# acappemin/Video-to-Audio-and-Piano-RP

Measured on AMD Instinct MI355X. Metric: mel-frames/sec (10s VGGSound shape, 32-step CFM, CFG 2.0), higher is better.
Workload: dtype bf16x3; 1 GPU; BASELINE.json configs[1]: 1 clip(s)/GPU x 750 latent frames x 128 ch, 32-point sway grid = 31 CFG evaluations (62 DiT forwards), T5 context 16 tokens, V2A zero roll; clips_per_gpu=1, global_clips=1, parallelism=clip-sharded x1, 1 all-gather, hipgraph=True, schedule=three streams, side_streams=True, cascade_passes=1

## Files before the change

video-to-audio-and-piano-rp_amd/csrc/gemm_common.h:

```cpp
#pragma once
#include "v2a_common.h"
#include <stdlib.h>
#include <type_traits>

namespace v2a_detail {

struct GemmParams {
  const void* a[3];
  int64_t lda[3];
  int32_t kend[3];
  int32_t nseg;
  const void* w;
  int64_t ldw;
  const float* bias;
  int32_t M, N, K;
  void* out;
  int64_t ldo;
  bf16_t* out2;
  int64_t ldo2;
  const float* resid;
  int64_t ldr;
  const float* gate;
  const int32_t* step;
  int64_t gss, gbs;
  int32_t rpb;
  const float* rope;
  int32_t rope_cols, rope_pos_off;
  int32_t vec_epi;
  int32_t relu;
  const int32_t* a_rowoff;
  const int32_t* a_koff;
  const int32_t* o_rowoff;
  int32_t krot;
  const float* ngam;
  int64_t ngss, ngbs;
  int32_t nsw_row, nsw_off;
  float* ssq;
  int64_t ssq_ld;
  const float* rssq;
  int64_t rssq_ld;
  int32_t rssq_parts;
  float rnorm;
  int32_t xcd_gm, xcd_gn;
  struct Rect { int32_t m_lo, n_lo, cnt, hm; float rcp; } rect[8];
  int32_t nrect, tiles_m, tiles_n;
  int32_t out2_split, out_split;
  int64_t alo[3];
  int64_t out2_lo;
  int32_t s3_kl;
  int32_t dbg;
};

struct GemmTuning {
  int force_tile;
  int krot;
  int use_8phase;
  int min_tiles_8phase;
  int xcd_grid;
  int dbg;
};
extern GemmTuning g_gemm_tuning;
extern int g_attn_one_group_from;
extern int g_dwconv_rows_per_wave;
extern int g_probe_dbg;
extern int g_dwconv_stream;

int launch_gemm_8phase(const GemmParams& p, int epilogue, int out_dtype, hipStream_t stream);

inline void fill_tile_map(GemmParams& p, int BM, int BN) {
  p.tiles_m = (p.M + BM - 1) / BM;
  p.tiles_n = (p.N + BN - 1) / BN;
  const int gm = p.xcd_gm, gn = p.xcd_gn;
  p.nrect = gm * gn;
  for (int r = 0; r < p.nrect; ++r) {
    const int xm = r / gn, xn = r % gn;
    const int m_lo = xm * p.tiles_m / gm, m_hi = (xm + 1) * p.tiles_m / gm;
    const int n_lo = xn * p.tiles_n / gn, n_hi = (xn + 1) * p.tiles_n / gn;
    const int hm = m_hi - m_lo;
    p.rect[r].m_lo = m_lo;
    p.rect[r].n_lo = n_lo;
    p.rect[r].cnt = hm * (n_hi - n_lo);
    p.rect[r].hm = hm > 0 ? hm : 1;
    p.rect[r].rcp = 1.0f / (float)(hm > 0 ? hm : 1);
  }
}

}

namespace {

using v2a_detail::GemmParams;

__device__ __forceinline__ void tile_of_index(const GemmParams& p, int L, int& tm, int& tn) {
  tm = tn = 0;
#pragma unroll
  for (int r = 0; r < 8; ++r) {
    if (r < p.nrect) {
      const int cnt = p.rect[r].cnt;
      if (L >= 0 && L < cnt) {
        const int hm = p.rect[r].hm;
        int q = (int)((float)L * p.rect[r].rcp);
        int rem = L - q * hm;
        if (rem < 0) { --q; rem += hm; }
        else if (rem >= hm) { ++q; rem -= hm; }
        tn = p.rect[r].n_lo + q;
        tm = p.rect[r].m_lo + rem;
      }
      L -= cnt;
    }
  }
}
__device__ __forceinline__ void tile_of_block(const GemmParams& p, int bid, int& tm, int& tn) {
  const int nwg = p.tiles_m * p.tiles_n;
  const int q = nwg >> 3, r = nwg & 7, xcd = bid & 7;
  const int L = (xcd < r ? xcd * (q + 1) : r * (q + 1) + (xcd - r) * q) + (bid >> 3);
  tile_of_index(p, L, tm, tn);
}

__host__ __device__ constexpr bool is_glu(int epi) { return epi == V2A_EPI_GEGLU || epi == V2A_EPI_SWIGLU; }
template <int EPI, bool FAST> __device__ __forceinline__ float glu_act(float g) {
  if constexpr (EPI == V2A_EPI_SWIGLU) return FAST ? silu_f(g) : silu_exact_f(g);
  else return FAST ? gelu_fast_f(g) : gelu_erf_f(g);
}

template <typename T> struct TileCfg;
template <> struct TileCfg<bf16_t> {
  static constexpr int BK = 64;
  static constexpr int LDS_ROW = 64;
};
template <> struct TileCfg<float> {
  static constexpr int BK = 16;
  static constexpr int LDS_ROW = 20;
};

template <int ROWS, bool SRC_F32> struct StageBf16 {
  static constexpr int N = ROWS / 32;
  bf16x8 r[N];
  __device__ __forceinline__ void load(const void* base, int64_t ld, int row0, int rows_total, int k0, int tid) {
    const int chunk = tid & 7;
#pragma unroll
    for (int i = 0; i < N; ++i) {
      int row = row0 + (tid >> 3) + 32 * i;
      row = row < rows_total ? row : rows_total - 1;
      if constexpr (SRC_F32) {
        const float* p = reinterpret_cast<const float*>(base) + (int64_t)row * ld + k0 + chunk * 8;
        f32x4 lo = *reinterpret_cast<const f32x4*>(p);
        f32x4 hi = *reinterpret_cast<const f32x4*>(p + 4);
        bf16x8 v;
#pragma unroll
        for (int j = 0; j < 4; ++j) {
          v[j] = (bf16_t)lo[j];
          v[4 + j] = (bf16_t)hi[j];
        }
        r[i] = v;
      } else {
        const bf16_t* p = reinterpret_cast<const bf16_t*>(base) + (int64_t)row * ld + k0 + chunk * 8;
        r[i] = *reinterpret_cast<const bf16x8*>(p);
      }
    }
  }
  __device__ __forceinline__ void store(bf16_t* lds, int tid) const {
    const int chunk = tid & 7;
#pragma unroll
    for (int i = 0; i < N; ++i) {
      int row = (tid >> 3) + 32 * i;
      *reinterpret_cast<bf16x8*>(lds + row * 64 + ((chunk ^ (row & 7)) << 3)) = r[i];
    }
  }
};

template <int ROWS> struct StageF32 {
  static constexpr int N = ROWS / 64;
  f32x4 r[N];
  __device__ __forceinline__ void load(const void* base, int64_t ld, int row0, int rows_total, int k0, int tid) {
    const int c4 = tid & 3;
#pragma unroll
    for (int i = 0; i < N; ++i) {
      int row = row0 + (tid >> 2) + 64 * i;
      row = row < rows_total ? row : rows_total - 1;
      const float* p = reinterpret_cast<const float*>(base) + (int64_t)row * ld + k0 + c4 * 4;
      r[i] = *reinterpret_cast<const f32x4*>(p);
    }
  }
  __device__ __forceinline__ void store(float* lds, int tid) const {
    const int c4 = tid & 3;
#pragma unroll
    for (int i = 0; i < N; ++i) {
      int row = (tid >> 2) + 64 * i;
      *reinterpret_cast<f32x4*>(lds + row * 20 + c4 * 4) = r[i];
    }
  }
};

template <typename T, bool A_F32, int ROWS> struct StageSel;
template <bool A_F32, int ROWS> struct StageSel<bf16_t, A_F32, ROWS> { using type = StageBf16<ROWS, A_F32>; };
template <bool A_F32, int ROWS> struct StageSel<float, A_F32, ROWS> { using type = StageF32<ROWS>; };

template <int EPI, typename OutT, int TM, int TN, int WM, int WN>
__device__ __forceinline__ void gemm_epilogue(const GemmParams& p, f32x4 (&acc)[TM][TN], int m0, int n0, int wm, int wn,
                                              int lr, int lq) {
  OutT* out = reinterpret_cast<OutT*>(p.out);
#pragma unroll
  for (int i = 0; i < TM; ++i) {
#pragma unroll
    for (int jj = 0; jj < 4; ++jj) {
      const int m = m0 + wm * WM + i * 16 + lq * 4 + jj;
      if (m >= p.M) continue;
      const float* gvec = nullptr;
      if constexpr (EPI == V2A_EPI_GATE_RESID) gvec = step_vec(p.gate, p.step, p.gss, p.gbs, p.gbs ? m / p.rpb : 0);
      if constexpr (is_glu(EPI)) {
#pragma unroll
        for (int j = 0; j < TN; j += 2) {
          const int n = n0 + wn * WN + j * 16 + lr;
          if (n >= p.N) continue;
          float v = acc[i][j][jj], g = acc[i][j + 1][jj];
          if (p.bias) { v += p.bias[n]; g += p.bias[n + 16]; }
          const int oc = ((n0 + wn * WN) >> 1) + (j >> 1) * 16 + lr;
          const float ge = glu_act<EPI, sizeof(OutT) == 2>(g);
          out[(int64_t)m * p.ldo + oc] = from_f32<OutT>(v * ge);
        }
      } else {
#pragma unroll
        for (int j = 0; j < TN; ++j) {
          const int n = n0 + wn * WN + j * 16 + lr;
          if (n >= p.N) continue;
          float v = acc[i][j][jj];
          if (p.bias) v += p.bias[n];
          if constexpr (EPI == V2A_EPI_SIGMOID) v = sigmoid_f(v);
          if constexpr (EPI == V2A_EPI_GELU) v = gelu_erf_f(v);
          if constexpr (EPI == V2A_EPI_RESID) v += p.resid[(int64_t)m * p.ldr + n];
          if constexpr (EPI == V2A_EPI_GATE_RESID) v = p.resid[(int64_t)m * p.ldr + n] + gvec[n] * v;
          if (p.relu) v = fmaxf(v, 0.f);
          out[(int64_t)m * p.ldo + n] = from_f32<OutT>(v);
          if constexpr (sizeof(OutT) == 4) {
            if (p.out2) p.out2[(int64_t)m * p.ldo2 + n] = (bf16_t)v;
          }
        }
      }
    }
  }
}


template <int EPI, int TM, int WN, bool ON> struct EpiPrefetch {
  static constexpr int LPR = WN / 4, RPI = 64 / LPR, RPS = 16 / RPI;
  static constexpr bool RES = ON && (EPI == V2A_EPI_RESID || EPI == V2A_EPI_GATE_RESID);
  static constexpr bool GATE = ON && EPI == V2A_EPI_GATE_RESID;
  f32x4 rs[RES ? TM : 1][RES ? RPS : 1];
  f32x4 gt[GATE ? TM : 1][GATE ? RPS : 1];
  static constexpr bool SCAT = RES && !GATE;
  int32_t ro[SCAT ? TM : 1][SCAT ? RPS : 1];
  static constexpr bool ROPE = ON && EPI == V2A_EPI_STORE;
  f32x4 cs[ROPE ? TM : 1][ROPE ? RPS : 1];
  __device__ __forceinline__ void load(const GemmParams& p, int m_base, int n_base, int lane) {
    if constexpr (ROPE) {
      const int c4 = (lane % LPR) * 4, r0 = lane / LPR;
      const int n = n_base + c4;
      if (p.rope && n < p.rope_cols) {
#pragma unroll
        for (int i = 0; i < TM; ++i)
#pragma unroll
          for (int q = 0; q < RPS; ++q) {
            int m = m_base + i * 16 + r0 + q * RPI;
            m = m < p.M ? m : p.M - 1;
            const int pos = p.rope_pos_off + m % p.rpb;
            cs[i][q] = *reinterpret_cast<const f32x4*>(p.rope + ((int64_t)pos * 32 + ((n & 63) >> 1)) * 2);
          }
      }
    }
    if constexpr (RES) {
      const int c4 = (lane % LPR) * 4, r0 = lane / LPR;
      const int n = n_base + c4;
      const int M = p.M;
      const bool full = n + 3 < p.N;
      const bool has_res = p.resid != nullptr, has_gate = p.gate != nullptr;
      const float* resid = p.resid + n;
      const int64_t ldr = p.ldr;
      const int32_t* orow = SCAT ? p.o_rowoff : nullptr;
      if constexpr (SCAT) {
        if (orow) {
#pragma unroll
          for (int i = 0; i < TM; ++i)
#pragma unroll
            for (int q = 0; q < RPS; ++q) {
              int m = m_base + i * 16 + r0 + q * RPI;
              m = m < M ? m : M - 1;
              ro[i][q] = orow[m];
            }
        }
      }
#pragma unroll
      for (int i = 0; i < TM; ++i)
#pragma unroll
        for (int q = 0; q < RPS; ++q) {
          const int m = m_base + i * 16 + r0 + q * RPI;
          if (m < M && full) {
            int64_t off = (int64_t)m * ldr;
            if constexpr (SCAT) { if (orow) off = ro[i][q]; }
            rs[i][q] = has_res ? *reinterpret_cast<const f32x4*>(resid + off) : f32x4{0.f, 0.f, 0.f, 0.f};
            if constexpr (GATE) gt[i][q] = has_gate ? *reinterpret_cast<const f32x4*>(step_vec(p.gate, p.step, p.gss, p.gbs, p.gbs ? m / p.rpb : 0) + n) : f32x4{1.f, 1.f, 1.f, 1.f};
          }
        }
    }
  }
};

constexpr int kRowSsqMax = 40;
struct RowScaleLoad {
  f32x4 v[kRowSsqMax / 4];
};
__device__ __forceinline__ void rowscale_load(const GemmParams& p, int m, RowScaleLoad& r) {
  m = m < p.M ? m : p.M - 1;
  const float* q = p.rssq + (int64_t)m * p.rssq_ld;
#pragma unroll
  for (int k = 0; k < kRowSsqMax / 4; ++k) {
    r.v[k] = f32x4{0.f, 0.f, 0.f, 0.f};
    if (4 * k < p.rssq_parts) r.v[k] = *reinterpret_cast<const f32x4*>(q + 4 * k);
  }
}
__device__ __forceinline__ float rowscale_finish(const GemmParams& p, const RowScaleLoad& r) {
  float s = 0.f;
#pragma unroll
  for (int k = 0; k < kRowSsqMax / 4; ++k) s += (r.v[k][0] + r.v[k][1]) + (r.v[k][2] + r.v[k][3]);
  return p.rnorm / fmaxf(sqrtf(s), 1e-12f);
}

__device__ __forceinline__ void rope_rotate4(f32x4& v, const f32x4& cs) {
  const float a0 = v[0], b0 = v[1], a1 = v[2], b1 = v[3];
  v[0] = fmaf(a0, cs[0], -(b0 * cs[1]));
  v[1] = fmaf(b0, cs[0], a0 * cs[1]);
  v[2] = fmaf(a1, cs[2], -(b1 * cs[3]));
  v[3] = fmaf(b1, cs[2], a1 * cs[3]);
}

template <int EPI, typename OutT, int TM, int TN, int WM, int WN, bool PF>
__device__ __forceinline__ void gemm_epilogue_lds(const GemmParams& p, f32x4 (&acc)[TM][TN], float* tile ,
                                                  int m_base, int n_base, int lane, const EpiPrefetch<EPI, TM, WN, PF>& pf,
                                                  const float* rs_row = nullptr ) {
  constexpr int LD = WN + 4;
  const int lr = lane & 15, lq = lane >> 4;
  OutT* out = reinterpret_cast<OutT*>(p.out);
  const int M = p.M;
  const bool relu = p.relu != 0;
  const int32_t* orow = p.o_rowoff;
  const int64_t ldo = p.ldo, ldr = p.ldr, ldo2 = p.ldo2;
  bf16_t* out2 = p.out2;
  const float* resid = p.resid;
  constexpr int LPRX = (is_glu(EPI) ? WN / 2 : WN) / 4;
  constexpr int RPSX = 16 / (64 / LPRX);
  f32x4 gmA = {1.f, 1.f, 1.f, 1.f}, gmB = gmA;
  if constexpr ((EPI == V2A_EPI_RESID || EPI == V2A_EPI_GATE_RESID) && sizeof(OutT) == 4) {
    const int nn = n_base + (lane % (WN / 4)) * 4;
    if (out2 && p.ngam && p.ngbs == 0 && nn + 3 < p.N) {
      const float* gb = step_vec(p.ngam, p.step, p.ngss, 0, 0) + nn;
      gmA = *reinterpret_cast<const f32x4*>(gb);
      gmB = *reinterpret_cast<const f32x4*>(gb + p.nsw_off);
    }
  }
  float rsc[TM][RPSX];
  const bool scaled = rs_row != nullptr;
  const bool geglu_wide = is_glu(EPI) && sizeof(OutT) == 2 && ((uintptr_t)p.out & 15) == 0 && (p.ldo & 7) == 0 && ((p.N >> 1) & 7) == 0 &&
                          !(p.dbg & 128);
  if (scaled) {
#pragma unroll
    for (int i = 0; i < TM; ++i)
#pragma unroll
      for (int q = 0; q < RPSX; ++q) rsc[i][q] = rs_row[i * 16 + lane / LPRX + q * (64 / LPRX)];
  }
#pragma unroll
  for (int i = 0; i < TM; ++i) {
    if (m_base + i * 16 >= M) continue;
#pragma unroll
    for (int j = 0; j < TN; ++j)
#pragma unroll
      for (int jj = 0; jj < 4; ++jj) tile[(lq * 4 + jj) * LD + j * 16 + lr] = acc[i][j][jj];
    if constexpr (is_glu(EPI) && sizeof(OutT) == 2 && (WN / 2) % 32 == 0) {
      if (geglu_wide) {
        constexpr int OC = WN / 2, LPR = OC / 8, RPI = 64 / LPR;
        static_assert(RPI <= 16, "one slab holds 16 rows");
        const int c8 = (lane % LPR) * 8, r0 = lane / LPR;
        const int lc = (c8 >> 4) * 32 + (c8 & 15);
        const int n = n_base + lc;
        f32x4 bv[2] = {{0.f, 0.f, 0.f, 0.f}, {0.f, 0.f, 0.f, 0.f}}, bg[2] = {{0.f, 0.f, 0.f, 0.f}, {0.f, 0.f, 0.f, 0.f}};
        if (p.bias && n < p.N) {
          bv[0] = *reinterpret_cast<const f32x4*>(p.bias + n);
          bv[1] = *reinterpret_cast<const f32x4*>(p.bias + n + 4);
          bg[0] = *reinterpret_cast<const f32x4*>(p.bias + n + 16);
          bg[1] = *reinterpret_cast<const f32x4*>(p.bias + n + 20);
        }
#pragma unroll
        for (int q = 0; q < 16 / RPI; ++q) {
          const int r = r0 + q * RPI;
          const int m = m_base + i * 16 + r;
          if (m >= p.M || n >= p.N) continue;
          const float rs = scaled ? rs_row[i * 16 + r] : 1.f;
          bf16x8 hi, lo;
#pragma unroll
          for (int h2 = 0; h2 < 2; ++h2) {
            f32x4 v = *reinterpret_cast<const f32x4*>(tile + r * LD + lc + 4 * h2);
            f32x4 g = *reinterpret_cast<const f32x4*>(tile + r * LD + lc + 16 + 4 * h2);
            if (scaled) {
              v *= rs;
              g *= rs;
            }
#pragma unroll
            for (int e = 0; e < 4; ++e) {
              const float o32 = (v[e] + bv[h2][e]) * glu_act<EPI, true>(g[e] + bg[h2][e]);
              hi[4 * h2 + e] = (bf16_t)o32;
              lo[4 * h2 + e] = (bf16_t)(o32 - (float)hi[4 * h2 + e]);
            }
          }
          OutT* dst = out + (int64_t)m * p.ldo + (n_base >> 1) + c8;
          *reinterpret_cast<bf16x8*>(dst) = hi;
          if (p.out_split) *reinterpret_cast<bf16x8*>(dst + (p.N >> 1)) = lo;
        }
        continue;
      }
    }
    if constexpr (is_glu(EPI)) {
      constexpr int OC = WN / 2;
      constexpr int LPR = OC / 4;
      constexpr int RPI = 64 / LPR;
      const int c4 = (lane % LPR) * 4, r0 = lane / LPR;
      const int lc = (c4 >> 4) * 32 + (c4 & 15);
      const int n = n_base + lc;
      f32x4 bv = {0.f, 0.f, 0.f, 0.f}, bg = {0.f, 0.f, 0.f, 0.f};
      if (p.bias && n < p.N) {
        bv = *reinterpret_cast<const f32x4*>(p.bias + n);
        bg = *reinterpret_cast<const f32x4*>(p.bias + n + 16);
      }
#pragma unroll
      for (int q = 0; q < 16 / RPI; ++q) {
        const int r = r0 + q * RPI;
        const int m = m_base + i * 16 + r;
        if (m >= p.M || n >= p.N) continue;
        f32x4 v = *reinterpret_cast<const f32x4*>(tile + r * LD + lc);
        f32x4 g = *reinterpret_cast<const f32x4*>(tile + r * LD + lc + 16);
        if (scaled) {
          v *= rsc[i][q];
          g *= rsc[i][q];
        }
        OutT* dst = out + (int64_t)m * p.ldo + (n_base >> 1) + c4;
        if constexpr (sizeof(OutT) == 2) {
          if (p.out_split) {
            bf16x4 hi, lo;
#pragma unroll
            for (int e = 0; e < 4; ++e) {
              const float o32 = (v[e] + bv[e]) * glu_act<EPI, true>(g[e] + bg[e]);
              hi[e] = (bf16_t)o32;
              lo[e] = (bf16_t)(o32 - (float)hi[e]);
            }
            *reinterpret_cast<bf16x4*>(dst) = hi;
            *reinterpret_cast<bf16x4*>(dst + (p.N >> 1)) = lo;
          } else {
            bf16x4 o;
#pragma unroll
            for (int e = 0; e < 4; ++e) o[e] = (bf16_t)((v[e] + bv[e]) * glu_act<EPI, true>(g[e] + bg[e]));
            *reinterpret_cast<bf16x4*>(dst) = o;
          }
        } else {
          f32x4 o;
#pragma unroll
          for (int e = 0; e < 4; ++e) o[e] = (v[e] + bv[e]) * glu_act<EPI, false>(g[e] + bg[e]);
          *reinterpret_cast<f32x4*>(dst) = o;
        }
      }
    } else {
      constexpr int LPR = WN / 4;
      constexpr int RPI = 64 / LPR;
      const int c4 = (lane % LPR) * 4, r0 = lane / LPR;
      const int n = n_base + c4;
      const bool full = n + 3 < p.N;
      f32x4 bv = {0.f, 0.f, 0.f, 0.f};
      if (p.bias && full) bv = *reinterpret_cast<const f32x4*>(p.bias + n);
#pragma unroll
      for (int q = 0; q < 16 / RPI; ++q) {
        const int r = r0 + q * RPI;
        const int m = m_base + i * 16 + r;
        if (m >= M || !full) continue;
        int64_t o_out = (int64_t)m * ldo, o_res = (int64_t)m * ldr, o_out2 = (int64_t)m * ldo2;
        if constexpr (EPI == V2A_EPI_STORE || EPI == V2A_EPI_RESID) {
          if (orow) {
            int64_t ro;
            if constexpr (PF && EPI == V2A_EPI_RESID) ro = pf.ro[i][q];
            else ro = orow[m];
            o_out = o_res = o_out2 = ro;
          }
        }
        f32x4 v = *reinterpret_cast<const f32x4*>(tile + r * LD + c4);
        if (scaled) v *= rsc[i][q];
#pragma unroll
        for (int e = 0; e < 4; ++e) v[e] += bv[e];
        if constexpr (EPI == V2A_EPI_SIGMOID) {
#pragma unroll
          for (int e = 0; e < 4; ++e) v[e] = sigmoid_f(v[e]);
        }
        if constexpr (EPI == V2A_EPI_GELU) {
#pragma unroll
          for (int e = 0; e < 4; ++e) v[e] = sizeof(OutT) == 2 ? gelu_fast_f(v[e]) : gelu_erf_f(v[e]);
        }
        if constexpr (EPI == V2A_EPI_STORE) {
          if (p.rope && n < p.rope_cols) {
            f32x4 cs;
            if constexpr (PF) cs = pf.cs[i][q];
            else cs = *reinterpret_cast<const f32x4*>(p.rope + ((int64_t)(p.rope_pos_off + m % p.rpb) * 32 + ((n & 63) >> 1)) * 2);
            rope_rotate4(v, cs);
          }
        }
        if constexpr (EPI == V2A_EPI_RESID || EPI == V2A_EPI_GATE_RESID) {
          f32x4 rs, gt = {1.f, 1.f, 1.f, 1.f};
          if constexpr (PF) {
            rs = pf.rs[i][q];
            if constexpr (EPI == V2A_EPI_GATE_RESID) gt = pf.gt[i][q];
          } else {
            rs = resid ? *reinterpret_cast<const f32x4*>(resid + o_res + n) : f32x4{0.f, 0.f, 0.f, 0.f};
            if constexpr (EPI == V2A_EPI_GATE_RESID) {
              if (p.gate) gt = *reinterpret_cast<const f32x4*>(step_vec(p.gate, p.step, p.gss, p.gbs, p.gbs ? m / p.rpb : 0) + n);
            }
          }
#pragma unroll
          for (int e = 0; e < 4; ++e) v[e] = rs[e] + gt[e] * v[e];
        }
        if (relu) {
#pragma unroll
          for (int e = 0; e < 4; ++e) v[e] = fmaxf(v[e], 0.f);
        }
        if constexpr (sizeof(OutT) == 2) {
          bf16x4 o;
#pragma unroll
          for (int e = 0; e < 4; ++e) o[e] = (bf16_t)v[e];
          *reinterpret_cast<bf16x4*>(out + o_out + n) = o;
          if constexpr (EPI == V2A_EPI_GELU) {
            if (p.out_split) {
              bf16x4 lo;
#pragma unroll
              for (int e = 0; e < 4; ++e) lo[e] = (bf16_t)(v[e] - (float)o[e]);
              *reinterpret_cast<bf16x4*>(out + o_out + p.N + n) = lo;
            }
          }
        } else {
          *reinterpret_cast<f32x4*>(out + o_out + n) = v;
          if (out2) {
            f32x4 gm = m >= p.nsw_row ? gmB : gmA;
            if (p.ngam && p.ngbs) gm = *reinterpret_cast<const f32x4*>(step_vec(p.ngam, p.step, p.ngss, p.ngbs, m / p.rpb) + (m >= p.nsw_row ? p.nsw_off : 0) + n);
            bf16x4 o;
#pragma unroll
            for (int e = 0; e < 4; ++e) o[e] = (bf16_t)(v[e] * gm[e]);
            *reinterpret_cast<bf16x4*>(out2 + o_out2 + n) = o;
            if (p.out2_split) {
              bf16x4 lo;
#pragma unroll
              for (int e = 0; e < 4; ++e) lo[e] = (bf16_t)(v[e] * gm[e] - (float)o[e]);
              *reinterpret_cast<bf16x4*>(out2 + o_out2 + p.out2_lo + n) = lo;
            }
            if (p.ssq) {
              const float ss = octet_sum(v[0] * v[0] + v[1] * v[1] + v[2] * v[2] + v[3] * v[3]);
              if ((lane & 7) == 0) p.ssq[(int64_t)m * p.ssq_ld + (n >> 5)] = ss;
            }
          }
        }
      }
    }
  }
}

}
```

Measured before the change: 3224 mel-frames/s.

## Software-pipeline GEMM epilogue loads and add unpredicated full-tile path

```diff
diff --git a/video-to-audio-and-piano-rp_amd/csrc/gemm_common.h b/video-to-audio-and-piano-rp_amd/csrc/gemm_common.h
--- a/video-to-audio-and-piano-rp_amd/csrc/gemm_common.h
+++ b/video-to-audio-and-piano-rp_amd/csrc/gemm_common.h
@@ -333,235 +333,372 @@
   v[3] = fmaf(b1, cs[2], a1 * cs[3]);
 }
 
+__device__ __forceinline__ void row_pos(int p0, int d, int rpb, bool multi, int& pos, int& nb) {
+  pos = p0 + d;
+  nb = 0;
+  if (pos >= rpb) { pos -= rpb; nb = 1; }
+  if (multi) {
+    while (pos >= rpb) { pos -= rpb; ++nb; }
+  }
+}
+
+template <int EPI, bool PF> constexpr bool epi_pipelined() { return !PF && (EPI == V2A_EPI_STORE || EPI == V2A_EPI_RESID || EPI == V2A_EPI_GATE_RESID); }
+
+template <int EPI, typename OutT, int TM, int TN, int WM, int WN, bool PF, bool ALL>
+__device__ __forceinline__ void gemm_epilogue_lds_impl(const GemmParams& p, f32x4 (&acc)[TM][TN], float* tile, int m_base, int n_base, int lane,
+                                                       const EpiPrefetch<EPI, TM, WN, PF>& pf, const float* rs_row) {
+  constexpr int LD = WN + 4;
+  const int lr = lane & 15, lq = lane >> 4;
+  OutT* out = reinterpret_cast<OutT*>(p.out);
+  const int M = p.M, N = p.N;
+  const bool relu = p.relu != 0;
+  const int32_t* orow = ALL ? nullptr : p.o_rowoff;
+  const int64_t ldo = p.ldo, ldr = p.ldr, ldo2 = p.ldo2;
+  bf16_t* out2 = p.out2;
+  const float* resid = p.resid;
+  const float* bias = p.bias;
+  constexpr int LPRX = (is_glu(EPI) ? WN / 2 : WN) / 4;
+  constexpr int RPSX = 16 / (64 / LPRX);
+  constexpr bool RESF = EPI == V2A_EPI_RESID || EPI == V2A_EPI_GATE_RESID;
+  constexpr bool GAMF = RESF && sizeof(OutT) == 4;
+  constexpr bool PIPE = epi_pipelined<EPI, PF>();
+  static_assert(PIPE || !ALL, "the unpredicated form belongs to the pipeline");
+  constexpr int LPRV = WN / 4, RPIV = 64 / LPRV, RPSV = 16 / RPIV;
+  const int c4v = (lane % LPRV) * 4, r0v = lane / LPRV;
+  const int nv = n_base + c4v;
+  const bool fullv = nv + 3 < N;
+  const bool scaled = rs_row != nullptr;
+  const bool geglu_wide = is_glu(EPI) && sizeof(OutT) == 2 && (WN / 2) % 32 == 0 && ((uintptr_t)p.out & 15) == 0 && (p.ldo & 7) == 0 &&
+                          ((p.N >> 1) & 7) == 0 && !(p.dbg & 128);
+
+  f32x4 bb[is_glu(EPI) ? 4 : 1];
+#pragma unroll
+  for (int k = 0; k < (is_glu(EPI) ? 4 : 1); ++k) bb[k] = f32x4{0.f, 0.f, 0.f, 0.f};
+  if constexpr (is_glu(EPI)) {
+    if (geglu_wide) {
+      const int c8 = (lane % (WN / 16)) * 8;
+      const int n = n_base + (c8 >> 4) * 32 + (c8 & 15);
+      if (bias && n < N) {
+        bb[0] = *reinterpret_cast<const f32x4*>(bias + n);
+        bb[1] = *reinterpret_cast<const f32x4*>(bias + n + 4);
+        bb[2] = *reinterpret_cast<const f32x4*>(bias + n + 16);
+        bb[3] = *reinterpret_cast<const f32x4*>(bias + n + 20);
+      }
+    } else {
+      const int c4 = (lane % (WN / 8)) * 4;
+      const int n = n_base + (c4 >> 4) * 32 + (c4 & 15);
+      if (bias && n < N) {
+        bb[0] = *reinterpret_cast<const f32x4*>(bias + n);
+        bb[2] = *reinterpret_cast<const f32x4*>(bias + n + 16);
+      }
+    }
+  } else {
+    if (bias && fullv) bb[0] = *reinterpret_cast<const f32x4*>(bias + nv);
+  }
+  const float* gate_b = nullptr;
+  const float* ngam_b = nullptr;
+  if constexpr (RESF) {
+    const int64_t stepv = p.step ? (int64_t)p.step[0] : 0;
+    if (p.gate) gate_b = p.gate + stepv * p.gss;
+    if (p.ngam) ngam_b = p.ngam + stepv * p.ngss;
+  }
+  const int rpb = p.rpb;
+  const bool rope_on = PIPE && EPI == V2A_EPI_STORE && p.rope != nullptr && n_base < p.rope_cols;
+  static_assert(64 % WN == 0 || EPI != V2A_EPI_STORE || PF, "a wave's columns lie in one 64-column head");
+  const bool gate_pb = PIPE && EPI == V2A_EPI_GATE_RESID && gate_b != nullptr && p.gbs != 0;
+  const bool gam_on = GAMF && out2 != nullptr && ngam_b != nullptr;
+  const bool gam_pb = gam_on && p.ngbs != 0;
+  int b0 = 0, p0 = 0;
+  bool onebatch = true, twobatch = true;
+  if (rope_on || gate_pb || (PIPE && gam_pb)) {
+    const int mb = __builtin_amdgcn_readfirstlane(m_base);
+    b0 = mb / rpb;
+    p0 = mb - b0 * rpb;
+    const int last = p0 + ((mb + WM < M ? mb + WM : M) - 1 - mb);
+    onebatch = last < rpb;
+    twobatch = last < 2 * rpb;
+  }
+  const int m_sw = m_base - p0 + rpb;
+  const bool multi = rpb < WM;
+  const bool gate_row = gate_pb && !twobatch, gam_row = gam_pb && !(PIPE && twobatch);
+  const bool gate_two = gate_pb && !onebatch && !gate_row, gam_two = PIPE && gam_pb && !onebatch && !gam_row;
+  f32x4 gmA = {1.f, 1.f, 1.f, 1.f}, gmB = gmA, gmC = gmA, gmD = gmA, gt1 = gmA, gt2 = gmA;
+  if constexpr (GAMF) {
+    if (gam_on && !gam_row && fullv && m_base < M) {
+      const float* gb = ngam_b + (gam_pb ? (int64_t)b0 * p.ngbs : 0) + nv;
+      gmA = *reinterpret_cast<const f32x4*>(gb);
+      gmB = *reinterpret_cast<const f32x4*>(gb + p.nsw_off);
+      if constexpr (PIPE) {
+        if (gam_two) {
+          gmC = *reinterpret_cast<const f32x4*>(gb + p.ngbs);
+          gmD = *reinterpret_cast<const f32x4*>(gb + p.ngbs + p.nsw_off);
+        }
+      }
+    }
+  }
+  if constexpr (PIPE && EPI == V2A_EPI_GATE_RESID) {
+    if (gate_b && !gate_row && fullv && m_base < M) {
+      const float* gp = gate_b + (gate_pb ? (int64_t)b0 * p.gbs : 0) + nv;
+      gt1 = *reinterpret_cast<const f32x4*>(gp);
+      if (gate_two) gt2 = *reinterpret_cast<const f32x4*>(gp + p.gbs);
+    }
+  }
+  float rsc[PIPE ? 1 : TM][PIPE ? 1 : RPSX];
+  if constexpr (!PIPE) {
+    if (scaled) {
+#pragma unroll
+      for (int i = 0; i < TM; ++i)
+#pragma unroll
+        for (int q = 0; q < RPSX; ++q) rsc[i][q] = rs_row[i * 16 + lane / LPRX + q * (64 / LPRX)];
+    }
+  }
+
+  f32x4 q_a[PIPE ? 2 : 1][PIPE ? RPSV : 1];
+  {
+#pragma unroll
+    for (int i = -1; i < TM; ++i) {
+      if (!ALL && m_base + (i < 0 ? 0 : i) * 16 >= M) break;
+      if constexpr (PIPE) {
+        if (i + 1 < TM && (ALL || m_base + (i + 1) * 16 < M)) {
+#pragma unroll
+          for (int q = 0; q < RPSV; ++q) {
+            const int m = m_base + (i + 1) * 16 + r0v + q * RPIV;
+            const bool ok = ALL || (m < M && fullv);
+            if constexpr (EPI == V2A_EPI_STORE) {
+              if (rope_on && ok) {
+                int pos, nb;
+                row_pos(p0, m - m_base, rpb, multi, pos, nb);
+                q_a[(i + 1) & 1][q] = *reinterpret_cast<const f32x4*>(p.rope + ((int64_t)(p.rope_pos_off + pos) * 32 + ((nv & 63) >> 1)) * 2);
+              }
+            }
+            if constexpr (RESF) {
+              if (ok) {
+                int64_t o_res = (int64_t)m * ldr;
+                if constexpr (EPI == V2A_EPI_RESID) { if (orow) o_res = orow[m]; }
+                q_a[(i + 1) & 1][q] = *reinterpret_cast<const f32x4*>(resid + o_res + nv);
+              }
+            }
+          }
+        }
+        __builtin_amdgcn_sched_barrier(0);
+      }
+      if (i < 0) continue;
+      if constexpr (PIPE) __builtin_amdgcn_sched_barrier(0);
+#pragma unroll
+      for (int j = 0; j < TN; ++j)
+#pragma unroll
+        for (int jj = 0; jj < 4; ++jj) tile[(lq * 4 + jj) * LD + j * 16 + lr] = acc[i][j][jj];
+      if (i == 0) {
+#pragma unroll
+        for (int k = 0; k < (is_glu(EPI) ? 4 : 1); ++k) asm volatile("" : "+v"(bb[k]));
+        if constexpr (GAMF) asm volatile("" : "+v"(gmA), "+v"(gmB), "+v"(gmC), "+v"(gmD));
+        if constexpr (PIPE && EPI == V2A_EPI_GATE_RESID) asm volatile("" : "+v"(gt1), "+v"(gt2));
+      }
+      if constexpr (is_glu(EPI) && sizeof(OutT) == 2 && (WN / 2) % 32 == 0) {
+        if (geglu_wide) {
+          constexpr int OC = WN / 2, LPR = OC / 8, RPI = 64 / LPR;
+          static_assert(RPI <= 16, "one slab holds 16 rows");
+          const int c8 = (lane % LPR) * 8, r0 = lane / LPR;
+          const int lc = (c8 >> 4) * 32 + (c8 & 15);
+          const int n = n_base + lc;
+#pragma unroll
+          for (int q = 0; q < 16 / RPI; ++q) {
+            const int r = r0 + q * RPI;
+            const int m = m_base + i * 16 + r;
+            if (m >= M || n >= N) continue;
+            const float rs = scaled ? rs_row[i * 16 + r] : 1.f;
+            bf16x8 hi, lo;
+#pragma unroll
+            for (int h2 = 0; h2 < 2; ++h2) {
+              f32x4 v = *reinterpret_cast<const f32x4*>(tile + r * LD + lc + 4 * h2);
+              f32x4 g = *reinterpret_cast<const f32x4*>(tile + r * LD + lc + 16 + 4 * h2);
+              if (scaled) {
+                v *= rs;
+                g *= rs;
+              }
+#pragma unroll
+              for (int e = 0; e < 4; ++e) {
+                const float o32 = (v[e] + bb[h2][e]) * glu_act<EPI, true>(g[e] + bb[2 + h2][e]);
+                hi[4 * h2 + e] = (bf16_t)o32;
+                lo[4 * h2 + e] = (bf16_t)(o32 - (float)hi[4 * h2 + e]);
+              }
+            }
+            OutT* dst = out + (int64_t)m * ldo + (n_base >> 1) + c8;
+            *reinterpret_cast<bf16x8*>(dst) = hi;
+            if (p.out_split) *reinterpret_cast<bf16x8*>(dst + (N >> 1)) = lo;
+          }
+          continue;
+        }
+      }
+      if constexpr (is_glu(EPI)) {
+        constexpr int OC = WN / 2;
+        constexpr int LPR = OC / 4;
+        constexpr int RPI = 64 / LPR;
+        const int c4 = (lane % LPR) * 4, r0 = lane / LPR;
+        const int lc = (c4 >> 4) * 32 + (c4 & 15);
+        const int n = n_base + lc;
+        const f32x4 bv = bb[0], bg = bb[2];
+#pragma unroll
+        for (int q = 0; q < 16 / RPI; ++q) {
+          const int r = r0 + q * RPI;
+          const int m = m_base + i * 16 + r;
+          if (m >= M || n >= N) continue;
+          f32x4 v = *reinterpret_cast<const f32x4*>(tile + r * LD + lc);
+          f32x4 g = *reinterpret_cast<const f32x4*>(tile + r * LD + lc + 16);
+          if (scaled) {
+            v *= rsc[i][q];
+            g *= rsc[i][q];
+          }
+          OutT* dst = out + (int64_t)m * ldo + (n_base >> 1) + c4;
+          if constexpr (sizeof(OutT) == 2) {
+            if (p.out_split) {
+              bf16x4 hi, lo;
+#pragma unroll
+              for (int e = 0; e < 4; ++e) {
+                const float o32 = (v[e] + bv[e]) * glu_act<EPI, true>(g[e] + bg[e]);
+                hi[e] = (bf16_t)o32;
+                lo[e] = (bf16_t)(o32 - (float)hi[e]);
+              }
+              *reinterpret_cast<bf16x4*>(dst) = hi;
+              *reinterpret_cast<bf16x4*>(dst + (N >> 1)) = lo;
+            } else {
+              bf16x4 o;
+#pragma unroll
+              for (int e = 0; e < 4; ++e) o[e] = (bf16_t)((v[e] + bv[e]) * glu_act<EPI, true>(g[e] + bg[e]));
+              *reinterpret_cast<bf16x4*>(dst) = o;
+            }
+          } else {
+            f32x4 o;
+#pragma unroll
+            for (int e = 0; e < 4; ++e) o[e] = (v[e] + bv[e]) * glu_act<EPI, false>(g[e] + bg[e]);
+            *reinterpret_cast<f32x4*>(dst) = o;
+          }
+        }
+      } else {
+        constexpr int RPI = RPIV;
+        const int c4 = c4v, r0 = r0v, n = nv;
+        const bool full = fullv;
+        const f32x4 bv = bb[0];
+#pragma unroll
+        for (int q = 0; q < 16 / RPI; ++q) {
+          const int r = r0 + q * RPI;
+          const int m = m_base + i * 16 + r;
+          if (!ALL && (m >= M || !full)) continue;
+          int64_t o_out = (int64_t)m * ldo, o_res = (int64_t)m * ldr, o_out2 = (int64_t)m * ldo2;
+          if constexpr (EPI == V2A_EPI_STORE || EPI == V2A_EPI_RESID) {
+            if (orow) {
+              int64_t ro;
+              if constexpr (PF && EPI == V2A_EPI_RESID) ro = pf.ro[i][q];
+              else ro = orow[m];
+              o_out = o_res = o_out2 = ro;
+            }
+          }
+          f32x4 v = *reinterpret_cast<const f32x4*>(tile + r * LD + c4);
+          if (scaled) v *= PIPE ? rs_row[i * 16 + r] : rsc[PIPE ? 0 : i][PIPE ? 0 : q];
+#pragma unroll
+          for (int e = 0; e < 4; ++e) v[e] += bv[e];
+          if constexpr (EPI == V2A_EPI_SIGMOID) {
+#pragma unroll
+            for (int e = 0; e < 4; ++e) v[e] = sigmoid_f(v[e]);
+          }
+          if constexpr (EPI == V2A_EPI_GELU) {
+#pragma unroll
+            for (int e = 0; e < 4; ++e) v[e] = sizeof(OutT) == 2 ? gelu_fast_f(v[e]) : gelu_erf_f(v[e]);
+          }
+          if constexpr (EPI == V2A_EPI_STORE) {
+            if constexpr (PF) {
+              if (p.rope && n < p.rope_cols) rope_rotate4(v, pf.cs[i][q]);
+            } else {
+              if (rope_on) rope_rotate4(v, q_a[i & 1][q]);
+            }
+          }
+          if constexpr (RESF) {
+            f32x4 rs, gt = {1.f, 1.f, 1.f, 1.f};
+            if constexpr (PF) {
+              rs = pf.rs[i][q];
+              if constexpr (EPI == V2A_EPI_GATE_RESID) gt = pf.gt[i][q];
+            } else {
+              rs = q_a[i & 1][q];
+              if constexpr (EPI == V2A_EPI_GATE_RESID) {
+                gt = gate_two && m >= m_sw ? gt2 : gt1;
+                if (gate_row) {
+                  int pos, nb;
+                  row_pos(p0, m - m_base, rpb, true, pos, nb);
+                  gt = *reinterpret_cast<const f32x4*>(gate_b + (int64_t)(b0 + nb) * p.gbs + n);
+                  asm volatile("" : "+v"(gt));
+                }
+              }
+            }
+#pragma unroll
+            for (int e = 0; e < 4; ++e) v[e] = rs[e] + gt[e] * v[e];
+          }
+          if (relu) {
+#pragma unroll
+            for (int e = 0; e < 4; ++e) v[e] = fmaxf(v[e], 0.f);
+          }
+          if constexpr (sizeof(OutT) == 2) {
+            bf16x4 o;
+#pragma unroll
+            for (int e = 0; e < 4; ++e) o[e] = (bf16_t)v[e];
+            *reinterpret_cast<bf16x4*>(out + o_out + n) = o;
+            if constexpr (EPI == V2A_EPI_GELU) {
+              if (p.out_split) {
+                bf16x4 lo;
+#pragma unroll
+                for (int e = 0; e < 4; ++e) lo[e] = (bf16_t)(v[e] - (float)o[e]);
+                *reinterpret_cast<bf16x4*>(out + o_out + N + n) = lo;
+              }
+            }
+          } else {
+            *reinterpret_cast<f32x4*>(out + o_out + n) = v;
+            if (out2) {
+              f32x4 gm = m >= p.nsw_row ? gmB : gmA;
+              if constexpr (GAMF) {
+                if constexpr (PIPE) {
+                  if (gam_two && m >= m_sw) gm = m >= p.nsw_row ? gmD : gmC;
+                }
+                if (gam_row) {
+                  int pos, nb = 0;
+                  if constexpr (PIPE) row_pos(p0, m - m_base, rpb, true, pos, nb);
+                  gm = *reinterpret_cast<const f32x4*>(ngam_b + (int64_t)(PIPE ? b0 + nb : m / rpb) * p.ngbs + (m >= p.nsw_row ? p.nsw_off : 0) + n);
+                  if constexpr (PIPE) asm volatile("" : "+v"(gm));
+                }
+              }
+              bf16x4 o;
+#pragma unroll
+              for (int e = 0; e < 4; ++e) o[e] = (bf16_t)(v[e] * gm[e]);
+              *reinterpret_cast<bf16x4*>(out2 + o_out2 + n) = o;
+              if (p.out2_split) {
+                bf16x4 lo;
+#pragma unroll
+                for (int e = 0; e < 4; ++e) lo[e] = (bf16_t)(v[e] * gm[e] - (float)o[e]);
+                *reinterpret_cast<bf16x4*>(out2 + o_out2 + p.out2_lo + n) = lo;
+              }
+              if (p.ssq) {
+                const float ss = octet_sum(v[0] * v[0] + v[1] * v[1] + v[2] * v[2] + v[3] * v[3]);
+                if ((lane & 7) == 0) p.ssq[(int64_t)m * p.ssq_ld + (n >> 5)] = ss;
+              }
+            }
+          }
+          if constexpr (PIPE) __builtin_amdgcn_sched_barrier(0);
+        }
+      }
+    }
+  }
+}
+
 template <int EPI, typename OutT, int TM, int TN, int WM, int WN, bool PF>
 __device__ __forceinline__ void gemm_epilogue_lds(const GemmParams& p, f32x4 (&acc)[TM][TN], float* tile ,
                                                   int m_base, int n_base, int lane, const EpiPrefetch<EPI, TM, WN, PF>& pf,
                                                   const float* rs_row = nullptr ) {
-  constexpr int LD = WN + 4;
-  const int lr = lane & 15, lq = lane >> 4;
-  OutT* out = reinterpret_cast<OutT*>(p.out);
-  const int M = p.M;
-  const bool relu = p.relu != 0;
-  const int32_t* orow = p.o_rowoff;
-  const int64_t ldo = p.ldo, ldr = p.ldr, ldo2 = p.ldo2;
-  bf16_t* out2 = p.out2;
-  const float* resid = p.resid;
-  constexpr int LPRX = (is_glu(EPI) ? WN / 2 : WN) / 4;
-  constexpr int RPSX = 16 / (64 / LPRX);
-  f32x4 gmA = {1.f, 1.f, 1.f, 1.f}, gmB = gmA;
-  if constexpr ((EPI == V2A_EPI_RESID || EPI == V2A_EPI_GATE_RESID) && sizeof(OutT) == 4) {
-    const int nn = n_base + (lane % (WN / 4)) * 4;
-    if (out2 && p.ngam && p.ngbs == 0 && nn + 3 < p.N) {
-      const float* gb = step_vec(p.ngam, p.step, p.ngss, 0, 0) + nn;
-      gmA = *reinterpret_cast<const f32x4*>(gb);
-      gmB = *reinterpret_cast<const f32x4*>(gb + p.nsw_off);
-    }
-  }
-  float rsc[TM][RPSX];
-  const bool scaled = rs_row != nullptr;
-  const bool geglu_wide = is_glu(EPI) && sizeof(OutT) == 2 && ((uintptr_t)p.out & 15) == 0 && (p.ldo & 7) == 0 && ((p.N >> 1) & 7) == 0 &&
-                          !(p.dbg & 128);
-  if (scaled) {
-#pragma unroll
-    for (int i = 0; i < TM; ++i)
-#pragma unroll
-      for (int q = 0; q < RPSX; ++q) rsc[i][q] = rs_row[i * 16 + lane / LPRX + q * (64 / LPRX)];
-  }
-#pragma unroll
-  for (int i = 0; i < TM; ++i) {
-    if (m_base + i * 16 >= M) continue;
-#pragma unroll
-    for (int j = 0; j < TN; ++j)
-#pragma unroll
-      for (int jj = 0; jj < 4; ++jj) tile[(lq * 4 + jj) * LD + j * 16 + lr] = acc[i][j][jj];
-    if constexpr (is_glu(EPI) && sizeof(OutT) == 2 && (WN / 2) % 32 == 0) {
-      if (geglu_wide) {
-        constexpr int OC = WN / 2, LPR = OC / 8, RPI = 64 / LPR;
-        static_assert(RPI <= 16, "one slab holds 16 rows");
-        const int c8 = (lane % LPR) * 8, r0 = lane / LPR;
-        const int lc = (c8 >> 4) * 32 + (c8 & 15);
-        const int n = n_base + lc;
-        f32x4 bv[2] = {{0.f, 0.f, 0.f, 0.f}, {0.f, 0.f, 0.f, 0.f}}, bg[2] = {{0.f, 0.f, 0.f, 0.f}, {0.f, 0.f, 0.f, 0.f}};
-        if (p.bias && n < p.N) {
-          bv[0] = *reinterpret_cast<const f32x4*>(p.bias + n);
-          bv[1] = *reinterpret_cast<const f32x4*>(p.bias + n + 4);
-          bg[0] = *reinterpret_cast<const f32x4*>(p.bias + n + 16);
-          bg[1] = *reinterpret_cast<const f32x4*>(p.bias + n + 20);
-        }
-#pragma unroll
-        for (int q = 0; q < 16 / RPI; ++q) {
-          const int r = r0 + q * RPI;
-          const int m = m_base + i * 16 + r;
-          if (m >= p.M || n >= p.N) continue;
-          const float rs = scaled ? rs_row[i * 16 + r] : 1.f;
-          bf16x8 hi, lo;
-#pragma unroll
-          for (int h2 = 0; h2 < 2; ++h2) {
-            f32x4 v = *reinterpret_cast<const f32x4*>(tile + r * LD + lc + 4 * h2);
-            f32x4 g = *reinterpret_cast<const f32x4*>(tile + r * LD + lc + 16 + 4 * h2);
-            if (scaled) {
-              v *= rs;
-              g *= rs;
-            }
-#pragma unroll
-            for (int e = 0; e < 4; ++e) {
-              const float o32 = (v[e] + bv[h2][e]) * glu_act<EPI, true>(g[e] + bg[h2][e]);
-              hi[4 * h2 + e] = (bf16_t)o32;
-              lo[4 * h2 + e] = (bf16_t)(o32 - (float)hi[4 * h2 + e]);
-            }
-          }
-          OutT* dst = out + (int64_t)m * p.ldo + (n_base >> 1) + c8;
-          *reinterpret_cast<bf16x8*>(dst) = hi;
-          if (p.out_split) *reinterpret_cast<bf16x8*>(dst + (p.N >> 1)) = lo;
-        }
-        continue;
-      }
-    }
-    if constexpr (is_glu(EPI)) {
-      constexpr int OC = WN / 2;
-      constexpr int LPR = OC / 4;
-      constexpr int RPI = 64 / LPR;
-      const int c4 = (lane % LPR) * 4, r0 = lane / LPR;
-      const int lc = (c4 >> 4) * 32 + (c4 & 15);
-      const int n = n_base + lc;
-      f32x4 bv = {0.f, 0.f, 0.f, 0.f}, bg = {0.f, 0.f, 0.f, 0.f};
-      if (p.bias && n < p.N) {
-        bv = *reinterpret_cast<const f32x4*>(p.bias + n);
-        bg = *reinterpret_cast<const f32x4*>(p.bias + n + 16);
-      }
-#pragma unroll
-      for (int q = 0; q < 16 / RPI; ++q) {
-        const int r = r0 + q * RPI;
-        const int m = m_base + i * 16 + r;
-        if (m >= p.M || n >= p.N) continue;
-        f32x4 v = *reinterpret_cast<const f32x4*>(tile + r * LD + lc);
-        f32x4 g = *reinterpret_cast<const f32x4*>(tile + r * LD + lc + 16);
-        if (scaled) {
-          v *= rsc[i][q];
-          g *= rsc[i][q];
-        }
-        OutT* dst = out + (int64_t)m * p.ldo + (n_base >> 1) + c4;
-        if constexpr (sizeof(OutT) == 2) {
-          if (p.out_split) {
-            bf16x4 hi, lo;
-#pragma unroll
-            for (int e = 0; e < 4; ++e) {
-              const float o32 = (v[e] + bv[e]) * glu_act<EPI, true>(g[e] + bg[e]);
-              hi[e] = (bf16_t)o32;
-              lo[e] = (bf16_t)(o32 - (float)hi[e]);
-            }
-            *reinterpret_cast<bf16x4*>(dst) = hi;
-            *reinterpret_cast<bf16x4*>(dst + (p.N >> 1)) = lo;
-          } else {
-            bf16x4 o;
-#pragma unroll
-            for (int e = 0; e < 4; ++e) o[e] = (bf16_t)((v[e] + bv[e]) * glu_act<EPI, true>(g[e] + bg[e]));
-            *reinterpret_cast<bf16x4*>(dst) = o;
-          }
-        } else {
-          f32x4 o;
-#pragma unroll
-          for (int e = 0; e < 4; ++e) o[e] = (v[e] + bv[e]) * glu_act<EPI, false>(g[e] + bg[e]);
-          *reinterpret_cast<f32x4*>(dst) = o;
-        }
-      }
-    } else {
-      constexpr int LPR = WN / 4;
-      constexpr int RPI = 64 / LPR;
-      const int c4 = (lane % LPR) * 4, r0 = lane / LPR;
-      const int n = n_base + c4;
-      const bool full = n + 3 < p.N;
-      f32x4 bv = {0.f, 0.f, 0.f, 0.f};
-      if (p.bias && full) bv = *reinterpret_cast<const f32x4*>(p.bias + n);
-#pragma unroll
-      for (int q = 0; q < 16 / RPI; ++q) {
-        const int r = r0 + q * RPI;
-        const int m = m_base + i * 16 + r;
-        if (m >= M || !full) continue;
-        int64_t o_out = (int64_t)m * ldo, o_res = (int64_t)m * ldr, o_out2 = (int64_t)m * ldo2;
-        if constexpr (EPI == V2A_EPI_STORE || EPI == V2A_EPI_RESID) {
-          if (orow) {
-            int64_t ro;
-            if constexpr (PF && EPI == V2A_EPI_RESID) ro = pf.ro[i][q];
-            else ro = orow[m];
-            o_out = o_res = o_out2 = ro;
-          }
-        }
-        f32x4 v = *reinterpret_cast<const f32x4*>(tile + r * LD + c4);
-        if (scaled) v *= rsc[i][q];
-#pragma unroll
-        for (int e = 0; e < 4; ++e) v[e] += bv[e];
-        if constexpr (EPI == V2A_EPI_SIGMOID) {
-#pragma unroll
-          for (int e = 0; e < 4; ++e) v[e] = sigmoid_f(v[e]);
-        }
-        if constexpr (EPI == V2A_EPI_GELU) {
-#pragma unroll
-          for (int e = 0; e < 4; ++e) v[e] = sizeof(OutT) == 2 ? gelu_fast_f(v[e]) : gelu_erf_f(v[e]);
-        }
-        if constexpr (EPI == V2A_EPI_STORE) {
-          if (p.rope && n < p.rope_cols) {
-            f32x4 cs;
-            if constexpr (PF) cs = pf.cs[i][q];
-            else cs = *reinterpret_cast<const f32x4*>(p.rope + ((int64_t)(p.rope_pos_off + m % p.rpb) * 32 + ((n & 63) >> 1)) * 2);
-            rope_rotate4(v, cs);
-          }
-        }
-        if constexpr (EPI == V2A_EPI_RESID || EPI == V2A_EPI_GATE_RESID) {
-          f32x4 rs, gt = {1.f, 1.f, 1.f, 1.f};
-          if constexpr (PF) {
-            rs = pf.rs[i][q];
-            if constexpr (EPI == V2A_EPI_GATE_RESID) gt = pf.gt[i][q];
-          } else {
-            rs = resid ? *reinterpret_cast<const f32x4*>(resid + o_res + n) : f32x4{0.f, 0.f, 0.f, 0.f};
-            if constexpr (EPI == V2A_EPI_GATE_RESID) {
-              if (p.gate) gt = *reinterpret_cast<const f32x4*>(step_vec(p.gate, p.step, p.gss, p.gbs, p.gbs ? m / p.rpb : 0) + n);
-            }
-          }
-#pragma unroll
-          for (int e = 0; e < 4; ++e) v[e] = rs[e] + gt[e] * v[e];
-        }
-        if (relu) {
-#pragma unroll
-          for (int e = 0; e < 4; ++e) v[e] = fmaxf(v[e], 0.f);
-        }
-        if constexpr (sizeof(OutT) == 2) {
-          bf16x4 o;
-#pragma unroll
-          for (int e = 0; e < 4; ++e) o[e] = (bf16_t)v[e];
-          *reinterpret_cast<bf16x4*>(out + o_out + n) = o;
-          if constexpr (EPI == V2A_EPI_GELU) {
-            if (p.out_split) {
-              bf16x4 lo;
-#pragma unroll
-              for (int e = 0; e < 4; ++e) lo[e] = (bf16_t)(v[e] - (float)o[e]);
-              *reinterpret_cast<bf16x4*>(out + o_out + p.N + n) = lo;
-            }
-          }
-        } else {
-          *reinterpret_cast<f32x4*>(out + o_out + n) = v;
-          if (out2) {
-            f32x4 gm = m >= p.nsw_row ? gmB : gmA;
-            if (p.ngam && p.ngbs) gm = *reinterpret_cast<const f32x4*>(step_vec(p.ngam, p.step, p.ngss, p.ngbs, m / p.rpb) + (m >= p.nsw_row ? p.nsw_off : 0) + n);
-            bf16x4 o;
-#pragma unroll
-            for (int e = 0; e < 4; ++e) o[e] = (bf16_t)(v[e] * gm[e]);
-            *reinterpret_cast<bf16x4*>(out2 + o_out2 + n) = o;
-            if (p.out2_split) {
-              bf16x4 lo;
-#pragma unroll
-              for (int e = 0; e < 4; ++e) lo[e] = (bf16_t)(v[e] * gm[e] - (float)o[e]);
-              *reinterpret_cast<bf16x4*>(out2 + o_out2 + p.out2_lo + n) = lo;
-            }
-            if (p.ssq) {
-              const float ss = octet_sum(v[0] * v[0] + v[1] * v[1] + v[2] * v[2] + v[3] * v[3]);
-              if ((lane & 7) == 0) p.ssq[(int64_t)m * p.ssq_ld + (n >> 5)] = ss;
-            }
-          }
-        }
-      }
-    }
-  }
-}
-
-}
+  if constexpr (epi_pipelined<EPI, PF>()) {
+    if (__builtin_amdgcn_readfirstlane((int)(m_base + WM <= p.M && n_base + WN <= p.N)) && p.o_rowoff == nullptr)
+      gemm_epilogue_lds_impl<EPI, OutT, TM, TN, WM, WN, PF, true>(p, acc, tile, m_base, n_base, lane, pf, rs_row);
+    else
+      gemm_epilogue_lds_impl<EPI, OutT, TM, TN, WM, WN, PF, false>(p, acc, tile, m_base, n_base, lane, pf, rs_row);
+  } else {
+    gemm_epilogue_lds_impl<EPI, OutT, TM, TN, WM, WN, PF, false>(p, acc, tile, m_base, n_base, lane, pf, rs_row);
+  }
+}
+
+}
```

New measurement: 3280 mel-frames/s, median of 6. +1.7%, better.
